# taleinat/fuzzysearch

Measured on NVIDIA H100. Metric: haystack_GB_per_s_scanned, higher is better.
Workload: dtype u8

## Files before the change

### fuzzysearch_b200/csrc/api.cu

```cuda
#include <algorithm>
#include <atomic>
#include <cstdarg>
#include <cstdio>
#include <cmath>
#include <cstring>
#include <dlfcn.h>
#include <sched.h>
#include <unistd.h>
#include <condition_variable>
#include <memory>
#include <mutex>
#include <thread>
#include <new>
#include <string>
#include <type_traits>
#include <vector>

#include "kernels.cuh"
#include "ham_kernels.cuh"
#include "lp_kernels.cuh"
#include "post_kernels.cuh"
#include "p2p_kernels.cuh"
#include "batch_kernels.cuh"
#include "ham_batch_kernels.cuh"
// ... 163 lines not shown
    int (*CommInitRank)(void **comm, int nranks, NcclId id, int rank) = nullptr;
    int (*AllGather)(const void *send, void *recv, size_t count, int dtype, void *comm, cudaStream_t s) = nullptr;
    int (*CommDestroy)(void *comm) = nullptr;
    const char *(*GetErrorString)(int) = nullptr;
    bool ok = false;
};
static NcclApi g_nccl;
static std::string g_nccl_path;

extern "C" void fzb_nccl_set_library(const char *path) { g_nccl_path = path ? path : ""; }

static int nccl_load() {
    static std::once_flag once;
    std::call_once(once, [] {
        void *lib = nullptr;
        if (!g_nccl_path.empty()) lib = dlopen(g_nccl_path.c_str(), RTLD_NOW | RTLD_GLOBAL);
        if (!lib) lib = dlopen("libnccl.so.2", RTLD_NOW | RTLD_GLOBAL);
        if (!lib) lib = dlopen("libnccl.so", RTLD_NOW | RTLD_GLOBAL);
        if (!lib) return;
        *(void **)&g_nccl.GetUniqueId = dlsym(lib, "ncclGetUniqueId");
        *(void **)&g_nccl.CommInitRank = dlsym(lib, "ncclCommInitRank");
        *(void **)&g_nccl.AllGather = dlsym(lib, "ncclAllGather");
        *(void **)&g_nccl.CommDestroy = dlsym(lib, "ncclCommDestroy");
        *(void **)&g_nccl.GetErrorString = dlsym(lib, "ncclGetErrorString");
        g_nccl.ok = g_nccl.GetUniqueId && g_nccl.CommInitRank && g_nccl.AllGather && g_nccl.CommDestroy;
    });
    return g_nccl.ok ? FZB_OK : fail(FZB_E_CUDA, "libnccl.so.2 not available: %s", dlerror() ? dlerror() : "missing symbols");
}

static void nccl_comm_destroy(void *comm) {
    if (g_nccl.ok && comm) g_nccl.CommDestroy(comm);
}

#define NCCLCK(call)                                                                                      \
    do {                                                                                                  \
        int r_ = (call);                                                                                  \
        if (r_ != 0)                                                                                      \
            return fail(FZB_E_CUDA, "%s failed: %s", #call, g_nccl.GetErrorString ? g_nccl.GetErrorString(r_) : "?"); \
    } while (0)

struct fzb_haystack {
    std::recursive_mutex mu;
    int device = 0;
    uint8_t *d = nullptr;
    DevBuf<uint8_t> owned_buf;
    uint64_t buf_len = 0, buf_lo = 0, global_len = 0, own_lo = 0, own_hi = 0;
    uint64_t padded_len = 0;
    cudaEvent_t ev_stop = nullptr;
    cudaStream_t stream = nullptr;
    DevBuf<uint32_t> d_bitmap;
    DevBuf<RawRec> d_out;
    DevBuf<uint32_t> d_counters;
    MappedBuf<uint32_t> h_counters;
    MappedBuf<int64_t> h_fin;
    DevBuf<int64_t> d_fin;
    DevBuf<uint64_t> d_sorted;
    fzb_result *pending = nullptr;
    bool ev1_recorded = false;
    bool filter_attrs_set = false;
    int scan_per_sm = 0;
    double coll_prob = -1.0;
    bool p2p = false;
    bool local_world = false;
    std::unique_ptr<PeerBufs> peer;
    uint8_t *peer_base[kMaxWorld] = {};
    bool peer_opened[kMaxWorld] = {};
    uint32_t p2p_cap = 4096;
    uint64_t slot_bytes = 0, flags_off = 0;
    uint32_t epoch = 0;
    bool counters_clean = false;
    uint32_t seq = 0;
    void *comm = nullptr;
    int rank = 0, world = 1;
    uint32_t gather_cap = 4096;
    std::unique_ptr<GatherBufs> gather;
    cudaEvent_t ev[4] = {nullptr, nullptr, nullptr, nullptr};
    int sm_count = 132;
    DevBuf<uint64_t> d_hits;
    DevBuf<uint32_t> d_glist;
    uint32_t glist_cap = 0;
    DevBuf<uint32_t> d_scratch;
    DevBuf<unsigned long long> d_lplist;
    std::unique_ptr<BatchBufs> batch;
    DevBuf<unsigned long long> d_mhits;
    std::unique_ptr<LpBatchBufs> lpb;
    std::unique_ptr<GenericBatchBufs> gbatch;
    std::unique_ptr<RecBufs> recs;
    std::unique_ptr<BestBufs> bestb;
    std::unique_ptr<NearBufs> nearb;
    std::unique_ptr<NearBatchBufs> nearbatch;
};

struct fzb_result {
    std::vector<RawRec> raw;
    uint32_t raw_n = 0;
    fzb_haystack *owner = nullptr;
    bool raw_in_stage = false;
    void fetch_raw();
    void discard_attempt();
    std::vector<RawRec> fin;
    std::vector<int64_t> hulls;
    bool unconsolidated = false;
    bool have_fin = false;
    bool device_post = false;
    bool raw_ordered = false;
    bool has_global = false;
    bool global_on_device = false;
    bool fused_issued = false;
    uint32_t fused_status = 0;
    uint32_t gcount = 0;
    std::vector<RawRec> gfin;
    int raw_order = 0;
    void order_raw();
    fzb_stats stats{};
};

static uint64_t round_up(uint64_t x, uint64_t a) { return (x + a - 1) / a * a; }

static RawRec make_rec(int64_t start, int64_t end, int64_t dist) {
    RawRec r;
    r.start = start;
    r.end = end;
    r.dist = (int32_t)dist;
    r.idx = -1;
    r.ngram = -1;
    return r;
}

struct HandleLock {
    std::recursive_mutex *m;
    explicit HandleLock(fzb_haystack *h) : m(h ? &h->mu : nullptr) {
        if (m) m->lock();
    }
    ~HandleLock() {
        if (m) m->unlock();
    }
    HandleLock(const HandleLock &) = delete;
    HandleLock &operator=(const HandleLock &) = delete;
};

static std::mutex g_pending_mutex;

void fzb_result::fetch_raw() {
    std::lock_guard<std::mutex> lock(g_pending_mutex);
    if (!owner) return;
    if (raw_in_stage) {
        raw.resize(raw_n);
        if (raw_n) {
            cudaSetDevice(owner->device);
            if (cudaMemcpyAsync(raw.data(), owner->d_out.get(), (size_t)raw_n * sizeof(RawRec), cudaMemcpyDeviceToHost,
                                owner->stream) != cudaSuccess ||
                cudaStreamSynchronize(owner->stream) != cudaSuccess) {
                cudaGetLastError();
                raw.clear();
                raw_n = 0;
            }
        }
        raw_in_stage = false;
    }
    if (global_on_device) {
        gfin.resize(gcount);
        for (uint32_t i = 0; i < gcount; i++) {
            const int64_t s0 = owner->peer->h_grows[2 * (size_t)i], v = owner->peer->h_grows[2 * (size_t)i + 1];
            gfin[i] = make_rec(s0, s0 + (v >> 32), v & 0xFFFFFFFF);
        }
        global_on_device = false;
    }
    owner->pending = nullptr;
    owner = nullptr;
}

void fzb_result::discard_attempt() {
    fetch_raw();
    raw.clear();
    raw_n = 0;
    fin.clear();
}

static void detach_pending(fzb_haystack *h) {
    fzb_result *r;
    {
        std::lock_guard<std::mutex> lock(g_pending_mutex);
        r = h->pending;
    }
    if (r) r->fetch_raw();
}

static int alloc_out(fzb_haystack *h, uint64_t cap) { return h->d_out.alloc(cap, cap * (sizeof(RawRec) + sizeof(uint64_t))); }

static int haystack_common_init(fzb_haystack *h) {
    CK(cudaSetDevice(h->device));
    CK(cudaStreamCreateWithFlags(&h->stream, cudaStreamNonBlocking));
    for (auto &e : h->ev) CK(cudaEventCreate(&e));
    CK(cudaEventCreate(&h->ev_stop));
    cudaDeviceProp prop;
    CK(cudaGetDeviceProperties(&prop, h->device));
    h->sm_count = prop.multiProcessorCount;
    uint64_t granules = (h->padded_len >> kGranuleShift) + 2;
    TRY(h->d_bitmap.alloc(round_up((granules + 31) / 32, 32)));
    TRY(h->d_counters.alloc(CNT_COUNT));
    TRY(h->h_counters.alloc(CNT_COUNT));
    memset(h->h_counters.get(), 0, CNT_COUNT * sizeof(uint32_t));
    TRY(h->h_fin.alloc((uint64_t)kPostMax * kFinCols));
    TRY(h->d_fin.alloc((uint64_t)kPostMax * kFinCols));
    TRY(h->d_sorted.alloc(kPostMax));
    CK(cudaFuncSetAttribute(k_post, cudaFuncAttributeMaxDynamicSharedMemorySize, (int)kPostSmem));
    CK(cudaMemset(h->d_bitmap.get(), 0, h->d_bitmap.size() * sizeof(uint32_t)));
    h->glist_cap = (uint32_t)std::min<uint64_t>(granules, 1u << 20);
    TRY(h->d_glist.alloc(std::max<uint32_t>(h->glist_cap, 1)));
    return alloc_out(h, 1u << 16);
}

static int check_shard(uint64_t buf_len, uint64_t buf_lo, uint64_t global_len, uint64_t own_lo,
                       uint64_t own_hi) {
    if (global_len >= (1ull << 46)) return fail(FZB_E_INVALID, "global_len must be below 2^46");
    if (buf_lo > global_len || buf_len > global_len - buf_lo || own_lo > own_hi || own_hi > global_len ||
        (own_lo < own_hi && (own_lo < buf_lo || own_hi > buf_lo + buf_len)))
        return fail(FZB_E_INVALID, "inconsistent shard geometry");
    if (buf_lo % 16 != 0) return fail(FZB_E_INVALID, "buf_lo must be a multiple of 16");
    if (buf_len >= (1ull << 40)) return fail(FZB_E_INVALID, "buf_len must be below 2^40");
    return FZB_OK;
}

static int alloc_buffer(fzb_haystack *h) {
    CK(cudaSetDevice(h->device));
    TRY(h->owned_buf.alloc(h->padded_len));
    h->d = h->owned_buf.get();
    CK(cudaMemset(h->d + h->buf_len, 0, h->padded_len - h->buf_len));
    return FZB_OK;
}

static void close_peers(fzb_haystack *h);
static int upload_bytes(fzb_haystack *h, uint64_t dst_off, const uint8_t *host, uint64_t n);

extern "C" void fzb_haystack_destroy(fzb_haystack *h) {
    if (!h) return;
    cudaSetDevice(h->device);
    if (h->stream) cudaStreamSynchronize(h->stream);
    detach_pending(h);
    if (h->comm) nccl_comm_destroy(h->comm);
    close_peers(h);
    for (auto &e : h->ev)
        if (e) cudaEventDestroy(e);
    if (h->ev_stop) cudaEventDestroy(h->ev_stop);
    if (h->stream) cudaStreamDestroy(h->stream);
    delete h;
}

static int haystack_new(const char *arg_error, const uint8_t *host, const void *dev_ptr, uint64_t buf_len,
                        uint64_t buf_lo, uint64_t global_len, uint64_t own_lo, uint64_t own_hi, int device,
                        fzb_haystack **out) {
    if (!out) return fail(FZB_E_INVALID, "out is NULL");
    *out = nullptr;
    if (arg_error) return fail(FZB_E_INVALID, "%s", arg_error);
    int rc = check_shard(buf_len, buf_lo, global_len, own_lo, own_hi);
    if (rc) return rc;
// ... 640 lines not shown
    uint64_t n = 0;
    for (uint64_t c : counts) n += c;
    std::vector<GroupRow> g;
    g.reserve(n);
    for (uint64_t c : counts) {
        const size_t seam = g.size();
        for (uint64_t i = 0; i < c; i++, rows += kFinCols) g.push_back(GroupRow{rows[0], rows[1], rows[2], rows[3], rows[4]});
        if (!std::is_sorted(g.begin() + seam, g.end(), group_less)) std::sort(g.begin() + seam, g.end(), group_less);
        if (seam > 0 && seam < g.size() && group_less(g[seam], g[seam - 1])) {
            auto lo = std::upper_bound(g.begin(), g.begin() + seam, g[seam], group_less);
            auto hi = std::lower_bound(g.begin() + seam, g.end(), g[seam - 1], group_less);
            std::inplace_merge(lo, g.begin() + seam, hi, group_less);
        }
    }
    if (!std::is_sorted(g.begin(), g.end(), group_less)) std::sort(g.begin(), g.end(), group_less);
    return g;
}

static void write_group_rows(const std::vector<RawRec> &fin, const std::vector<int64_t> &hulls, size_t n, int64_t *rows) {
    for (size_t i = 0; i < n; i++, rows += kFinCols) {
        rows[0] = fin[i].start;
        rows[1] = fin[i].end;
        rows[2] = fin[i].dist;
        rows[3] = hulls[2 * i];
        rows[4] = hulls[2 * i + 1];
    }
}

extern "C" int64_t fzb_consolidate(const int64_t *start, const int64_t *end, const int32_t *dist, uint64_t n,
                                   int64_t *out_start, int64_t *out_end, int32_t *out_dist) {
    if (n && (!start || !end || !dist)) return fail(FZB_E_INVALID, "NULL input");
    std::vector<RawRec> o;
    sweep_groups(match_rows(start, end, dist, n), o);
    for (size_t i = 0; i < o.size(); i++) {
        if (out_start) out_start[i] = o[i].start;
        if (out_end) out_end[i] = o[i].end;
        if (out_dist) out_dist[i] = o[i].dist;
    }
    return (int64_t)o.size();
}

extern "C" int64_t fzb_consolidate_groups(const int64_t *start, const int64_t *end, const int32_t *dist, uint64_t n,
                                          int64_t *out_rows) {
    if (n && (!start || !end || !dist || !out_rows)) return fail(FZB_E_INVALID, "NULL input");
    std::vector<RawRec> o;
    std::vector<int64_t> hulls;
    sweep_groups(match_rows(start, end, dist, n), o, &hulls);
    write_group_rows(o, hulls, o.size(), out_rows);
    return (int64_t)o.size();
}

extern "C" int64_t fzb_result_group_rows(const fzb_result *r, int64_t *rows, uint64_t max_rows) {
    if (!r || (!rows && max_rows)) return fail(FZB_E_INVALID, "NULL argument");
    if (!r->have_fin || r->hulls.size() != r->fin.size() * 2)
        return fail(FZB_E_INVALID, "result was produced with FZB_F_NO_FINAL");
    write_group_rows(r->fin, r->hulls, std::min<size_t>(r->fin.size(), max_rows), rows);
    return (int64_t)r->fin.size();
}

extern "C" int fzb_result_hulls(const fzb_result *r, int64_t *hull_start, int64_t *hull_end) {
    if (!r) return fail(FZB_E_INVALID, "result is NULL");
    if (!r->have_fin || r->hulls.size() != r->fin.size() * 2)
        return fail(FZB_E_INVALID, "result was produced with FZB_F_NO_FINAL");
    for (size_t i = 0; i < r->fin.size(); i++) {
        if (hull_start) hull_start[i] = r->hulls[2 * i];
        if (hull_end) hull_end[i] = r->hulls[2 * i + 1];
    }
    return FZB_OK;
}

extern "C" int64_t fzb_merge_groups(const int64_t *rows, uint64_t n, int64_t *out_start, int64_t *out_end,
                                    int32_t *out_dist) {
    if (n && !rows) return fail(FZB_E_INVALID, "NULL input");
    std::vector<RawRec> o;
    sweep_groups(read_group_runs(rows, {n}), o);
    for (size_t i = 0; i < o.size(); i++) {
        if (out_start) out_start[i] = o[i].start;
        if (out_end) out_end[i] = o[i].end;
        if (out_dist) out_dist[i] = o[i].dist;
    }
    return (int64_t)o.size();
}

static int allgather_groups_staged(fzb_haystack *h, const std::vector<int64_t> &rows, std::vector<int64_t> &all,
                                   std::vector<uint64_t> &counts) {
    const uint64_t n = rows.size() / kFinCols;
    for (;;) {
        const uint32_t cap = h->gather_cap;
        TRY(ensure_gather_buffers(h, cap));
        GatherBufs &g = *h->gather;
        const size_t slot_rows = (size_t)cap + 1, slot = slot_rows * kFinCols * sizeof(int64_t);
        g.h_send[0] = (int64_t)n;
        g.h_send[1] = n <= cap;
        g.h_send[2] = g.h_send[3] = g.h_send[4] = 0;
        if (n <= cap && n) memcpy(g.h_send.get() + kFinCols, rows.data(), n * kFinCols * sizeof(int64_t));
        CK(cudaMemcpyAsync(g.d_send.get(), g.h_send.get(), (1 + (n <= cap ? n : 0)) * kFinCols * sizeof(int64_t),
                           cudaMemcpyHostToDevice, h->stream));
        NCCLCK(g_nccl.AllGather(g.d_send.get(), g.d_recv.get(), slot,  0, h->comm, h->stream));
        CK(cudaMemcpyAsync(g.h_recv.get(), g.d_recv.get(), slot * h->world, cudaMemcpyDeviceToHost, h->stream));
        CK(cudaStreamSynchronize(h->stream));
        uint64_t top = 0;
        for (int r = 0; r < h->world; r++) top = std::max<uint64_t>(top, (uint64_t)g.h_recv[(size_t)r * slot_rows * kFinCols]);
        if (top <= cap) {
            all.clear();
            counts.clear();
            for (int r = 0; r < h->world; r++) {
                const int64_t *base = g.h_recv.get() + (size_t)r * slot_rows * kFinCols;
                all.insert(all.end(), base + kFinCols, base + kFinCols + (size_t)base[0] * kFinCols);
                counts.push_back((uint64_t)base[0]);
            }
            return FZB_OK;
        }
        while (h->gather_cap < top) h->gather_cap *= 2;
    }
// ... 109 lines not shown

constexpr uint64_t kMaxRawRecs = 1ull << 27;

static int ensure_out_cap(fzb_haystack *h, uint64_t need) {
    if (need <= h->d_out.size()) return FZB_OK;
    uint64_t cap = h->d_out.size();
    while (cap < need) cap *= 2;
    if (cap > kMaxRawRecs) return fail(FZB_E_UNSUPPORTED, "more than 2^27 raw matches in one search");
    return alloc_out(h, cap);
}


static int wait_done(fzb_haystack *h, const volatile uint32_t *word) {
    const uint32_t want = h->seq;
    for (uint64_t spins = 0; *word != want; spins++) {
#if defined(__x86_64__) || defined(__i386__)
        __builtin_ia32_pause();
#endif
        if ((spins & 0xFFF) == 0xFFF) {
            const cudaError_t e = cudaStreamQuery(h->stream);
            if (e == cudaSuccess) break;
            if (e != cudaErrorNotReady) return fail(FZB_E_CUDA, "search failed: %s", cudaGetErrorString(e));
        }
    }
    std::atomic_thread_fence(std::memory_order_acquire);
    if (*word != want) {
        CK(cudaStreamSynchronize(h->stream));
        CK(cudaGetLastError());
        if (*word != want) return fail(FZB_E_CUDA, "search kernels did not complete");
    }
    return FZB_OK;
}

struct PostPlan {
    int mode = 1;
    bool global = false;
};

static void finalize_on_host(fzb_result *res, int mode);

template <class F>
static int run_emitting(fzb_haystack *h, fzb_result *res, F enqueue, PostPlan post = PostPlan()) {
    detach_pending(h);
    for (int attempt = 0; attempt < 8; attempt++) {
        if (!h->counters_clean) CK(cudaMemsetAsync(h->d_counters.get(), 0, CNT_COUNT * sizeof(uint32_t), h->stream));
        h->counters_clean = false;
        CK(cudaEventRecord(h->ev[0], h->stream));
        h->ev1_recorded = false;
        int rc = enqueue();
        if (rc) return rc;
        CK(cudaGetLastError());
        h->seq++;
        PostArgs pa{reinterpret_cast<const uint64_t *>(h->d_out.get() + h->d_out.size()), (uint32_t)h->d_out.size(), post.mode,
                    h->d_sorted.get(), h->d_fin.get(), h->h_fin.get(), h->h_counters.get(), h->d_counters.get(), h->seq, 0};
        pa.clear = !(post.global && attempt == 0 && h->p2p && !res->fused_issued);
        k_post<<<h->sm_count, kPostThreads, kPostSmem, h->stream>>>(pa);
        CK(cudaGetLastError());
        res->stats.n_launches++;
        const bool fused = post.global && attempt == 0 && h->p2p && !res->fused_issued;
        if (fused) {
            h->epoch++;
            WorldArgs w{};
            w.world = h->world;
            w.rank = h->rank;
            w.epoch = h->epoch;
            w.cap = h->p2p_cap;
            w.slot_bytes = h->slot_bytes;
            w.flags_off = h->flags_off;
            for (int r = 0; r < h->world; r++) w.peer[r] = h->peer_base[r];
            PeerBufs &pb = *h->peer;
            k_push<<<kPushCtas, kPushThreads, 0, h->stream>>>(w, h->d_fin.get(), h->d_counters.get(), post.mode, pb.d_ms.get());
            MergeOut mo{pb.d_mscore.get(), pb.d_mpos.get(), pb.h_grows.get(), pb.h_ghdr.get(), h->seq};
            k_merge<<<h->world, kPostThreads, 0, h->stream>>>(w, pb.d_ms.get(), mo);
            CK(cudaGetLastError());
            res->stats.n_launches += 2;
        }
        CK(cudaEventRecord(h->ev[2], h->stream));
        rc = wait_done(h, fused ? h->peer->h_ghdr.get() + 7 : h->h_counters.get() + CNT_SEQ);
        if (rc) return rc;
        const uint32_t n = h->h_counters[CNT_OUT];
        res->stats.n_candidates = h->h_counters[CNT_CAND];
        if (fused) {
            res->fused_issued = true;
            res->fused_status = h->peer->h_ghdr[0];
            res->gcount = h->peer->h_ghdr[1];
            if (h->peer->h_ghdr[2] != h->epoch && res->fused_status == MS_OK) res->fused_status = MS_TIMEOUT;
        }
        if (n > h->d_out.size()) {
            TRY(ensure_out_cap(h, n));
            continue;
        }
        const bool posted = h->h_counters[CNT_POST_DONE] != 0;
        h->counters_clean = posted && (!fused || (res->fused_status == MS_OK));
        res->raw.clear();
        res->raw_n = n;
        res->raw_ordered = false;
        if (posted || (res->fused_issued && res->fused_status == MS_OK)) {
            std::lock_guard<std::mutex> lock(g_pending_mutex);
            res->raw_in_stage = posted;
            res->owner = h;
            h->pending = res;
        }
        if (!posted && n) {
            res->raw.resize(n);
            CK(cudaMemcpyAsync(res->raw.data(), h->d_out.get(), (size_t)n * sizeof(RawRec), cudaMemcpyDeviceToHost, h->stream));
            CK(cudaStreamSynchronize(h->stream));
        }
        res->fin.clear();
        res->hulls.clear();
        res->have_fin = false;
        res->device_post = false;
        if (post.mode != 0) {
            if (posted) {
                const uint32_t nf = h->h_counters[CNT_NFINAL];
                res->fin.resize(nf);
                res->hulls.resize((size_t)nf * 2);
                for (uint32_t i = 0; i < nf; i++) {
                    res->fin[i] = make_rec(h->h_fin[kFinCols * i], h->h_fin[kFinCols * i + 1], h->h_fin[kFinCols * i + 2]);
                    res->hulls[2 * i] = h->h_fin[kFinCols * i + 3];
                    res->hulls[2 * i + 1] = h->h_fin[kFinCols * i + 4];
                }
                res->device_post = true;
            } else {
                finalize_on_host(res, post.mode);
            }
            res->have_fin = true;
        }
        float ms = 0.f;
        while (cudaEventQuery(h->ev[2]) == cudaErrorNotReady) {
        }
        cudaEventElapsedTime(&ms, h->ev[0], h->ev[2]);
        res->stats.gpu_ms = ms;
        res->stats.filter_ms = ms;
        if (h->ev1_recorded) {
            cudaEventElapsedTime(&ms, h->ev[0], h->ev[1]);
            res->stats.filter_ms = ms;
        }
        return FZB_OK;
    }
    return fail(FZB_E_CUDA, "output buffer kept overflowing");
}

static void sort_generation_order(std::vector<RawRec> &v) {
    std::sort(v.begin(), v.end(), [](const RawRec &a, const RawRec &b) {
        if (a.ngram != b.ngram) return a.ngram < b.ngram;
        return a.idx < b.idx;
    });
}

static void sort_canonical(std::vector<RawRec> &v) {
    std::sort(v.begin(), v.end(), [](const RawRec &a, const RawRec &b) {
        if (a.start != b.start) return a.start < b.start;
        if (a.end != b.end) return a.end < b.end;
        return a.dist < b.dist;
    });
}

void fzb_result::order_raw() {
    fetch_raw();
    if (raw_ordered) return;
    if (raw_order == 0)
        sort_generation_order(raw);
    else if (raw_order == 1)
        sort_canonical(raw);
    else
        std::sort(raw.begin(), raw.end(), [](const RawRec &a, const RawRec &b) {
            if (a.ngram != b.ngram) return a.ngram < b.ngram;
            if (a.idx != b.idx) return a.idx < b.idx;
            if (a.start != b.start) return a.start < b.start;
            if (a.end != b.end) return a.end < b.end;
            return a.dist < b.dist;
        });
    raw_ordered = true;
}

static void finalize_on_host(fzb_result *res, int mode) {
    if (mode == 1) {
        consolidate_recs(res->raw, res->fin, &res->hulls);
        return;
    }
    res->fin = res->raw;
    sort_canonical(res->fin);
    res->hulls.resize(res->fin.size() * 2);
    for (size_t i = 0; i < res->fin.size(); i++) {
        res->fin[i].idx = -1;
        res->fin[i].ngram = -1;
        res->hulls[2 * i] = res->fin[i].start;
        res->hulls[2 * i + 1] = res->fin[i].end;
    }
}

static int set_filter_attrs(size_t smem) {
    CK(cudaFuncSetAttribute(k_filter_sampled, cudaFuncAttributeMaxDynamicSharedMemorySize, (int)smem));
    CK(cudaFuncSetAttribute(k_filter_dense<0>, cudaFuncAttributeMaxDynamicSharedMemorySize, (int)kDenseSmem));
    CK(cudaFuncSetAttribute(k_filter_dense<1>, cudaFuncAttributeMaxDynamicSharedMemorySize, (int)kDenseSmem));
    CK(cudaFuncSetAttribute(k_filter_dense<2>, cudaFuncAttributeMaxDynamicSharedMemorySize, (int)kDenseSmem));
    CK(cudaFuncSetAttribute(k_filter_dense<3>, cudaFuncAttributeMaxDynamicSharedMemorySize, (int)kDenseSmem));
    CK(cudaFuncSetAttribute(k_filter_dense2, cudaFuncAttributeMaxDynamicSharedMemorySize, (int)kDense2Smem));
    return FZB_OK;
}

constexpr int kVerifyCtasPerSm = 8;

static bool sampled_filter_applies(uint32_t m, uint32_t k, uint32_t flags) {
    if (flags & FZB_F_FORCE_DENSE) return false;
    if (m < 4 || m < k + 3) return false;
    return (m - k - 3) / 4 >= k + 1;
}

static int sample_collision_prob(fzb_haystack *h) {
    if (h->coll_prob >= 0.0) return FZB_OK;
    const uint64_t blk = 4096, nblk = 16;
// ... 261 lines not shown
                k_generic_lp<R><<<grid, kLpThreads, 0, h->stream>>>(p, h->d_scratch.get(), cap, h->d_out.get(),
                                                                    h->d_out.size(), h->d_counters.get(), rs);
            });
            res->stats.n_launches++;
            return FZB_OK;
        }, PostPlan{post_mode, post_mode != 0 && (flags & FZB_F_GLOBAL) != 0});
        if (rc) return rc;
        res->raw_order = 1;
        return FZB_OK;
    }
    p.L = (int)pl.L();
    p.n_ngrams = (int)pl.m / p.L;
    const bool sampled = sampled_filter(h, pl, flags);
    p.q = sampled ? 4 : std::min(p.L, 8);
    res->stats.route = 5;
    rc = set_filter_attrs(kScanSmem);
    if (rc) return rc;
    rc = run_lp(h, res, [&](int grid, int cap) -> int {
        int r2 = enqueue_filter(h, p, sampled, res);
        if (r2) return r2;
        with_recs(h, [&](auto rec) {
            constexpr bool R = decltype(rec)::value;
            k_verify_generic<R><<<grid, kLpThreads, 0, h->stream>>>(p, h->d_bitmap.size(), h->d_scratch.get(), cap,
                                                                    h->d_out.get(), h->d_out.size(), h->d_counters.get(), rs);
        });
        res->stats.n_launches++;
        return FZB_OK;
    }, PostPlan{post_mode, post_mode != 0 && (flags & FZB_F_GLOBAL) != 0});
    if (rc) return rc;
    res->raw_order = 2;
    return FZB_OK;
}

static int finish_global(fzb_haystack *h, fzb_result *res) {
    if (h->world < 1 || (!h->comm && !h->local_world))
        return fail(FZB_E_INVALID, "FZB_F_GLOBAL needs fzb_haystack_comm_init / fzb_comm_init_local");
    if (res->fused_issued) {
        if (res->fused_status == MS_OK) {
            res->has_global = true;
            res->global_on_device = true;
            return FZB_OK;
        }
        if (res->fused_status == MS_TIMEOUT)
            return fail(FZB_E_CUDA, "multi-GPU reduction timed out waiting for a peer (rank %d of %d)", h->rank, h->world);
    }
    if (h->local_world && res->fused_issued && res->fused_status == MS_OVERFLOW)
        return fail(FZB_E_UNSUPPORTED, "NCCL-free world: more than %u groups continue across shard seams; the staged "
                    "fallback needs an NCCL communicator (fzb_haystack_comm_init)", kMaxNonHeads);
    if (h->local_world)
        return fail(FZB_E_UNSUPPORTED, "NCCL-free world: a shard produced more than %u groups (or more than %d raw "
                    "matches); the staged fallback needs an NCCL communicator (fzb_haystack_comm_init)", h->p2p_cap, kPostMax);
    std::vector<int64_t> all;
    std::vector<uint64_t> counts;
    std::vector<int64_t> rows(res->fin.size() * kFinCols);
    write_group_rows(res->fin, res->hulls, res->fin.size(), rows.data());
    int rc = allgather_groups_staged(h, rows, all, counts);
    if (rc) return rc;
    if (res->unconsolidated) {
        res->gfin.resize(all.size() / kFinCols);
        for (size_t i = 0; i < res->gfin.size(); i++)
            res->gfin[i] = make_rec(all[kFinCols * i], all[kFinCols * i + 1], all[kFinCols * i + 2]);
        sort_canonical(res->gfin);
    } else {
        sweep_groups(read_group_runs(all.data(), counts), res->gfin);
    }
    res->gcount = (uint32_t)res->gfin.size();
    res->has_global = true;
    return FZB_OK;
}

static int make_result(fzb_result **out, fzb_result **res) {
    if (!out) return fail(FZB_E_INVALID, "out is NULL");
    *out = nullptr;
    *res = new (std::nothrow) fzb_result();
    if (!*res) return fail(FZB_E_CUDA, "out of host memory");
    return FZB_OK;
}

static int search_hamming(fzb_haystack *h, const uint8_t *pattern, const Plan &pl, uint32_t flags, fzb_result *res);

static int run_route(fzb_haystack *h, const uint8_t *pattern, const Plan &pl, uint32_t flags, fzb_result *res) {
    res->unconsolidated = pl.route == Route::Exact || pl.route == Route::Hamming;
    const int post_mode = res->unconsolidated ? 2 : (flags & FZB_F_NO_FINAL) ? 0 : 1;
    int rc = pl.route == Route::Hamming ? search_hamming(h, pattern, pl, flags, res)
             : pl.route == Route::LevLp ? search_lev_lp(h, pattern, pl, flags, res, post_mode)
             : pl.generic()             ? search_generic(h, pattern, pl, flags, res, post_mode)
                                        : search_lev_ngrams(h, pattern, pl, flags, res, post_mode);
    if (rc == FZB_OK && post_mode && (flags & FZB_F_GLOBAL)) rc = finish_global(h, res);
    return rc;
}

template <class P>
static int run_search(fzb_haystack *h, const uint8_t *pattern, uint32_t flags, fzb_result **out, P plan) {
    HandleLock handle_lock(h);
    fzb_result *res;
    int rc = make_result(out, &res);
    if (rc) return rc;
    Plan pl;
    rc = plan(pl);
    if (rc == FZB_OK) rc = run_route(h, pattern, pl, flags, res);
    if (rc) {
        fzb_result_destroy(res);
        return rc;
    }
    *out = res;
    return FZB_OK;
// ... 755 lines not shown
    explicit BufferView(fzb_haystack *hs)
        : h(hs), d(hs->d), buf_len(hs->buf_len), buf_lo(hs->buf_lo), own_lo(hs->own_lo), own_hi(hs->own_hi),
          padded_len(hs->padded_len), global_len(hs->global_len), coll_prob(hs->coll_prob) {}
    ~BufferView() {
        h->d = d;
        h->buf_len = buf_len;
        h->buf_lo = buf_lo;
        h->own_lo = own_lo;
        h->own_hi = own_hi;
        h->padded_len = padded_len;
        h->global_len = global_len;
        h->coll_prob = coll_prob;
    }
    BufferView(const BufferView &) = delete;
    BufferView &operator=(const BufferView &) = delete;
    void set(uint64_t vlo, uint64_t vhi, uint64_t lo, uint64_t hi) {
        h->d = d + (vlo - buf_lo);
        h->buf_lo = vlo;
        h->buf_len = vhi - vlo;
        h->padded_len = round_up(h->buf_len, 128) + 128;
        h->own_lo = lo;
        h->own_hi = hi;
    }
};

extern "C" int fzb_search_exact_window(fzb_haystack *h, const uint8_t *pattern, uint32_t m, uint64_t start,
                                       uint64_t end, uint32_t flags, fzb_result **out) {
    HandleLock handle_lock(h);
    if (!h || !out) return fail(FZB_E_INVALID, "NULL argument");
    *out = nullptr;
    TRY(refuse_records(h, "the windowed exact search"));
    if (flags & FZB_F_GLOBAL) return fail(FZB_E_INVALID, "windowed exact search is per handle");
    if (!is_whole_sequence(h)) return fail(FZB_E_INVALID, "windowed exact search needs a whole (unsharded) sequence");
    start = std::min<uint64_t>(start, h->global_len);
    end = std::max<uint64_t>(start, std::min<uint64_t>(end, h->global_len));
    if (end - start < m) {
        Plan pl;
        int rc0 = plan_exact(h, pattern, m, flags, pl);
        if (rc0) return rc0;
        fzb_result *res;
        rc0 = make_result(out, &res);
        if (rc0) return rc0;
        res->unconsolidated = true;
        res->have_fin = true;
        *out = res;
        return FZB_OK;
    }
    const uint64_t halo = round_up((uint64_t)m, 128) + 128;
    BufferView view(h);
    view.set((start > halo ? start - halo : 0) / 128 * 128, end, start, end);
    h->global_len = end;
    h->coll_prob = -1.0;
    const int rc = fzb_search_exact(h, pattern, m, flags, out);
    if (rc == FZB_OK && *out) (*out)->fetch_raw();
    return rc;
}

typedef CUresult (*EncodeTiledFn)(CUtensorMap *, CUtensorMapDataType, cuuint32_t, void *, const cuuint64_t *,
                                  const cuuint64_t *, const cuuint32_t *, const cuuint32_t *, CUtensorMapInterleave,
                                  CUtensorMapSwizzle, CUtensorMapL2promotion, CUtensorMapFloatOOBfill);

static int make_row_maps(fzb_haystack *h, CUtensorMap *map256, CUtensorMap *map8) {
    static const EncodeTiledFn encode = []() -> EncodeTiledFn {
        void *fn = nullptr;
        cudaDriverEntryPointQueryResult q;
        if (cudaGetDriverEntryPoint("cuTensorMapEncodeTiled", &fn, cudaEnableDefault, &q) != cudaSuccess) return nullptr;
        return (fn && q == cudaDriverEntryPointSuccess) ? (EncodeTiledFn)fn : nullptr;
    }();
    if (!encode) {
        cudaGetLastError();
        return fail(FZB_E_CUDA, "cuTensorMapEncodeTiled not available");
    }
    const cuuint64_t rows = h->padded_len / kHcRowBytes;
    const cuuint64_t dims[2] = {(cuuint64_t)kHcRowBytes, rows};
    const cuuint64_t strides[1] = {(cuuint64_t)kHcRowBytes};
    const cuuint32_t estr[2] = {1, 1};
    for (int which = 0; which < 2; which++) {
        const cuuint32_t box[2] = {(cuuint32_t)kHcRowBytes, which == 0 ? 256u : (cuuint32_t)kHcHaloRows};
        CUresult r = encode(which == 0 ? map256 : map8, CU_TENSOR_MAP_DATA_TYPE_UINT8, 2, h->d, dims, strides, box,
                            estr, CU_TENSOR_MAP_INTERLEAVE_NONE, CU_TENSOR_MAP_SWIZZLE_128B,
                            CU_TENSOR_MAP_L2_PROMOTION_L2_128B, CU_TENSOR_MAP_FLOAT_OOB_FILL_NONE);
        if (r != CUDA_SUCCESS) return fail(FZB_E_CUDA, "cuTensorMapEncodeTiled failed (%d)", (int)r);
    }
    return FZB_OK;
}

static int search_hamming(fzb_haystack *h, const uint8_t *pattern, const Plan &pl, uint32_t flags, fzb_result *res) {
    const uint32_t m = pl.m;
    int rc;
    ScanParams p;
    fill_params(h, pattern, m, p);
    p.k = (int)pl.k;
    if (flags & FZB_F_TINY_LIST) p.glist_cap = std::min(h->glist_cap, 8u);
    const RecSet rs = rec_set(h);
    CK(cudaSetDevice(h->device));
    res->stats.route = 4;
    res->stats.bytes_scanned = h->buf_len;
    const bool counting = !(flags & FZB_F_FORCE_DENSE) && (int)m >= 4 * p.k + 7 && p.k <= 7 && h->buf_len > 0;
    HamCountParams hp{};
    CUtensorMap map256, map8;
    int slices = 0;
    if (counting) {
        hp.Wc = std::min<int>((int)(m - 3) / 4, 8);
        slices = hp.Wc - p.k <= 4 ? 2 : 3;
        hp.bias = (1 << slices) - (hp.Wc - p.k);
        hp.nrows = (int64_t)(round_up(h->buf_len, kHcRowBytes) / kHcRowBytes);
        rc = make_row_maps(h, &map256, &map8);
// ... 931 lines not shown
    } while (rc == FZB_OK && !*found && lo < whole.own_hi);
    return rc;
}

extern "C" int fzb_debug_counters(const fzb_haystack *h, uint32_t out[32]) {
    if (!h || !out) return fail(FZB_E_INVALID, "NULL argument");
    memset(out, 0, 32 * sizeof(uint32_t));
    memcpy(out, h->h_counters.get(), CNT_COUNT * sizeof(uint32_t));
    if (h->peer) memcpy(out + 16, h->peer->h_ghdr.get(), 16 * sizeof(uint32_t));
    return FZB_OK;
}

extern "C" int fzb_debug_expand(const uint8_t *subs, const uint32_t *sub_off, const uint8_t *seqs,
                                const uint32_t *seq_off, const int32_t *max_l, const int32_t *variant, uint32_t count,
                                int device, int32_t *out) {
    if (count && (!subs || !sub_off || !seqs || !seq_off || !max_l || !variant || !out))
        return fail(FZB_E_INVALID, "NULL argument");
    if (device < 0 || device >= fzb_device_count()) return fail(FZB_E_CUDA, "CUDA device %d not available", device);
    if (count == 0) return FZB_OK;
    for (uint32_t i = 0; i < count; i++) {
        if (sub_off[i + 1] < sub_off[i] || seq_off[i + 1] < seq_off[i]) return fail(FZB_E_INVALID, "bad offsets");
        if (sub_off[i + 1] - sub_off[i] >= (uint32_t)kDbgMax || seq_off[i + 1] - seq_off[i] >= 2u * kDbgMax)
            return fail(FZB_E_UNSUPPORTED, "case %u too long for the debug entry", i);
        if (variant[i] < 0 || variant[i] > 2 || max_l[i] < 0) return fail(FZB_E_INVALID, "bad variant / budget");
    }
    CK(cudaSetDevice(device));
    const size_t nsub = std::max<size_t>(sub_off[count], 1), nseq = std::max<size_t>(seq_off[count], 1);
    DevBuf<uint8_t> d_subs, d_seqs;
    DevBuf<uint32_t> d_so, d_qo;
    DevBuf<int32_t> d_k, d_v, d_out;
    TRY(d_subs.alloc(nsub));
    TRY(d_seqs.alloc(nseq));
    TRY(d_so.alloc(count + 1));
    TRY(d_qo.alloc(count + 1));
    TRY(d_k.alloc(count));
    TRY(d_v.alloc(count));
    TRY(d_out.alloc((uint64_t)count * 8));
    CK(cudaMemcpy(d_subs.get(), subs, sub_off[count], cudaMemcpyHostToDevice));
    CK(cudaMemcpy(d_seqs.get(), seqs, seq_off[count], cudaMemcpyHostToDevice));
    CK(cudaMemcpy(d_so.get(), sub_off, (count + 1) * sizeof(uint32_t), cudaMemcpyHostToDevice));
    CK(cudaMemcpy(d_qo.get(), seq_off, (count + 1) * sizeof(uint32_t), cudaMemcpyHostToDevice));
    CK(cudaMemcpy(d_k.get(), max_l, count * sizeof(int32_t), cudaMemcpyHostToDevice));
    CK(cudaMemcpy(d_v.get(), variant, count * sizeof(int32_t), cudaMemcpyHostToDevice));
    k_debug_expand<<<count, 32>>>(d_subs.get(), d_so.get(), d_seqs.get(), d_qo.get(), d_k.get(), d_v.get(), d_out.get());
    CK(cudaGetLastError());
    CK(cudaMemcpy(out, d_out.get(), (size_t)count * 8 * sizeof(int32_t), cudaMemcpyDeviceToHost));
    return FZB_OK;
}

extern "C" uint64_t fzb_result_count(const fzb_result *r, int which) {
    if (!r) return 0;
    if (which != FZB_RAW && r->has_global) return r->gcount;
    if (which == FZB_RAW) return r->raw_n;
    return r->fin.size();
}

extern "C" int fzb_result_copy(const fzb_result *r, int which, int64_t *start, int64_t *end, int32_t *dist,
                               int32_t *anchor_ngram, int64_t *anchor_idx) {
    if (!r) return fail(FZB_E_INVALID, "result is NULL");
    if (which == FZB_RAW) const_cast<fzb_result *>(r)->order_raw();
    if (which != FZB_RAW && r->has_global) const_cast<fzb_result *>(r)->fetch_raw();
    const std::vector<RawRec> &v = (which != FZB_RAW && r->has_global) ? r->gfin : (which == FZB_RAW ? r->raw : r->fin);
    const bool anchors = (which == FZB_RAW) && (r->stats.route <= 2);
    for (size_t i = 0; i < v.size(); i++) {
        if (start) start[i] = v[i].start;
        if (end) end[i] = v[i].end;
        if (dist) dist[i] = v[i].dist;
        if (anchor_ngram) anchor_ngram[i] = anchors ? v[i].ngram : -1;
        if (anchor_idx) anchor_idx[i] = anchors ? v[i].idx : -1;
    }
    return FZB_OK;
}

extern "C" int fzb_result_stats(const fzb_result *r, fzb_stats *out) {
    if (!r || !out) return fail(FZB_E_INVALID, "NULL argument");
    *out = r->stats;
    return FZB_OK;
}

extern "C" void fzb_result_destroy(fzb_result *r) {
    if (!r) return;
    {
        std::lock_guard<std::mutex> lock(g_pending_mutex);
        if (r->owner) {
            r->owner->pending = nullptr;
            r->owner = nullptr;
        }
    }
    delete r;
}
```

### fuzzysearch_b200/csrc/post_kernels.cuh

```cuda
#pragma once
#include "kernels.cuh"

namespace fzb {

constexpr int kPostMax = 16384;
constexpr int kPostThreads = 1024;
enum { CNT_POST_DONE = 5, CNT_NFINAL = 6, CNT_TICKET = 9, CNT_SEQ = 15 };
constexpr int kFinCols = 5;
constexpr size_t kPostSmem = (size_t)kPostMax * 8 + (size_t)kPostMax * 4;

struct PostArgs {
    const uint64_t *rkeys;
    uint32_t cap;
    int mode;
    uint64_t *sorted;
    int64_t *fin;
    int64_t *h_fin;
    uint32_t *h_counters;
    uint32_t *counters;
    uint32_t seq;
    int clear;
};

__device__ __forceinline__ uint32_t gtimer_lo() {
#ifdef FZB_EMU
    return (uint32_t)emu::cycles();
#else
    unsigned long long t;
    asm volatile("mov.u64 %0, %globaltimer;" : "=l"(t));
    return (uint32_t)t;
#endif
}

__device__ __forceinline__ uint32_t block_scan_sum(uint32_t v, uint32_t *scratch, uint32_t *total) {
    const int lane = threadIdx.x & 31, w = threadIdx.x >> 5;
    uint32_t inc = v;
#pragma unroll
    for (int o = 1; o < 32; o <<= 1) {
        const uint32_t t = __shfl_up_sync(0xFFFFFFFFu, inc, o);
        if (lane >= o) inc += t;
    }
    if (lane == 31) scratch[w] = inc;
    __syncthreads();
    if (w == 0) {
        const uint32_t x = scratch[lane];
        uint32_t xi = x;
#pragma unroll
        for (int o = 1; o < 32; o <<= 1) {
            const uint32_t t = __shfl_up_sync(0xFFFFFFFFu, xi, o);
            if (lane >= o) xi += t;
        }
        scratch[lane] = xi - x;
        if (lane == 31) scratch[32] = xi;
    }
    __syncthreads();
    const uint32_t r = scratch[w] + inc - v;
    *total = scratch[32];
    __syncthreads();
    return r;
}

__device__ __forceinline__ unsigned long long block_scan_max(unsigned long long v, unsigned long long *scratch,
                                                             unsigned long long *total) {
    const int lane = threadIdx.x & 31, w = threadIdx.x >> 5;
    unsigned long long inc = v;
#pragma unroll
    for (int o = 1; o < 32; o <<= 1) {
        const unsigned long long t = __shfl_up_sync(0xFFFFFFFFu, inc, o);
        if (lane >= o) inc = max(inc, t);
    }
// ... 31 lines not shown
    __shared__ uint32_t s_ticket;
    const uint32_t nraw = a.counters[CNT_OUT];
    const uint32_t n = a.counters[CNT_KEYS];
    const bool fits = nraw <= (uint32_t)kPostMax && nraw <= a.cap;
    const uint32_t tid = threadIdx.x, lane = tid & 31, warp = tid >> 5;
    const uint32_t G = gridDim.x, b = blockIdx.x;
    if (!fits) {
        if (b == 0) {
            if (tid < CNT_SEQ) a.h_counters[tid] = a.counters[tid];
            __threadfence_system();
            __syncthreads();
            if (tid == 0) a.h_counters[CNT_SEQ] = a.seq;
        }
        return;
    }
    const uint32_t t_start = gtimer_lo();
    const uint32_t lo = (uint32_t)((uint64_t)n * b / G), hi = (uint32_t)((uint64_t)n * (b + 1) / G);
    if (a.mode != 0 && n > 0) {
        for (uint32_t i = tid; i < n; i += kPostThreads) keys[i] = a.rkeys[i];
        __syncthreads();
        for (uint32_t i0 = lo + 2 * warp; i0 < hi; i0 += 2 * (kPostThreads / 32)) {
            const uint32_t i1 = min(i0 + 1, hi - 1);
            const uint64_t key0 = keys[i0], key1 = keys[i1];
            uint32_t c0 = 0, c1 = 0;
            for (uint32_t j = lane; j < n; j += 32) {
                const uint64_t kj = keys[j];
                c0 += (kj < key0) || (kj == key0 && j < i0);
                c1 += (kj < key1) || (kj == key1 && j < i1);
            }
            c0 = __reduce_add_sync(0xFFFFFFFFu, c0);
            c1 = __reduce_add_sync(0xFFFFFFFFu, c1);
            if (lane == 0) {
                a.sorted[c0] = key0;
                a.sorted[c1] = key1;
            }
        }
    }
    const uint32_t t_ranked = gtimer_lo();
    __threadfence();
    __syncthreads();
    if (tid == 0) s_ticket = atomicAdd(&a.counters[CNT_TICKET], 1u);
    __syncthreads();
    if (s_ticket != G - 1) return;
    __threadfence();
    const uint32_t t_ticket = gtimer_lo();
    uint32_t t_sorted = t_ticket, t_swept = t_ticket;
    uint32_t nfinal = 0;
    if (a.mode != 0 && n > 0) {
        for (uint32_t i = tid; i < n; i += kPostThreads) keys[i] = __ldcg(a.sorted + i);
        __syncthreads();
        t_sorted = gtimer_lo();
        if (a.mode == 2) {
            nfinal = n;
            for (uint32_t i = tid; i < n; i += kPostThreads) {
                const uint64_t kx = keys[i];
                const int64_t s = (int64_t)(kx >> 18), e = s + (int64_t)((kx >> 8) & 1023u);
                int64_t *row = a.fin + (size_t)kFinCols * i;
                row[0] = s;
                row[1] = e;
                row[2] = (int64_t)(kx & 255u);
                row[3] = s;
                row[4] = e;
            }
        } else {
            for (uint32_t i = tid; i < n; i += kPostThreads) segbest[i] = 0xFFFFFFFFu;
            __syncthreads();
            unsigned long long carry_hull = 0;
            uint32_t carry_groups = 0;
            for (uint32_t base = 0; base < n; base += kPostThreads) {
                const uint32_t i = base + tid;
                const bool live = i < n;
                const uint64_t kx = live ? keys[i] : 0;
                const unsigned long long s = kx >> 18, len = (kx >> 8) & 1023u, e = live ? s + len : 0;
                unsigned long long round_max;
                const unsigned long long hull = max(carry_hull, block_scan_max(e, scr64, &round_max));
                const bool head = live && (i == 0 || s >= hull);
                uint32_t round_heads;
                const uint32_t before = block_scan_sum(head ? 1u : 0u, scr32, &round_heads);
                if (live) {
                    const uint32_t g = carry_groups + before + (head ? 1u : 0u) - 1u;
                    if (head) {
                        a.fin[(size_t)kFinCols * g + 3] = (int64_t)s;
                        if (g >= 1) a.fin[(size_t)kFinCols * (g - 1) + 4] = (int64_t)hull;
                    }
                    if (i == n - 1) a.fin[(size_t)kFinCols * g + 4] = (int64_t)max(hull, e);
                    const uint32_t score = ((uint32_t)(kx & 255u) << 24) | ((uint32_t)(1023u - len) << 14) | i;
                    atomicMin(&segbest[g], score);
                }
                carry_hull = max(carry_hull, round_max);
                carry_groups += round_heads;
            }
            nfinal = carry_groups;
            __syncthreads();
            for (uint32_t g = tid; g < nfinal; g += kPostThreads) {
                const uint64_t kx = keys[segbest[g] & 16383u];
                const int64_t s = (int64_t)(kx >> 18);
                int64_t *row = a.fin + (size_t)kFinCols * g;
                row[0] = s;
                row[1] = s + (int64_t)((kx >> 8) & 1023u);
                row[2] = (int64_t)(kx & 255u);
            }
        }
        __threadfence_block();
        __syncthreads();
        t_swept = gtimer_lo();
        const uint32_t nvec = (uint32_t)(((size_t)nfinal * kFinCols * 8 + 15) / 16);
        const uint4 *src = reinterpret_cast<const uint4 *>(a.fin);
        uint4 *dst = reinterpret_cast<uint4 *>(a.h_fin);
        for (uint32_t i = tid; i < nvec; i += kPostThreads) dst[i] = __ldcg(src + i);
    }
    __syncthreads();
    if (tid == 0) {
        a.counters[CNT_NFINAL] = nfinal;
        a.counters[CNT_POST_DONE] = 1u;
        a.counters[10] = t_ranked - t_start;
        a.counters[11] = t_sorted - t_ranked;
        a.counters[12] = t_swept - t_sorted;
        a.counters[13] = gtimer_lo() - t_swept;
    }
    __syncthreads();
    if (tid < CNT_SEQ) a.h_counters[tid] = a.counters[tid];
    if (a.clear && tid < CNT_COUNT) a.counters[tid] = 0;
    __threadfence_system();
    __syncthreads();
    if (tid == 0) a.h_counters[CNT_SEQ] = a.seq;
}

}
```

Measured before the change: 2782.

## Stage compact keys to host and defer hull rows fetch lazily

The post kernel now writes one packed 64-bit key per final match to mapped host memory, replacing the 5-column int64 rows it used to copy. Hull rows stay in device memory and are pulled only when a caller asks for groups or hulls. Result decoding on the host is deferred until first access. The segment sweep is also changed from many block-wide scan rounds to one chunked per-thread pass with a single max-scan and sum-scan, cutting __syncthreads rounds. The cost is extra complexity in the lazy fetch state and a synchronous device copy when hulls are requested.

```diff
diff --git a/fuzzysearch_b200/csrc/api.cu b/fuzzysearch_b200/csrc/api.cu
--- a/fuzzysearch_b200/csrc/api.cu
+++ b/fuzzysearch_b200/csrc/api.cu
@@ -239,7 +239,7 @@
     DevBuf<RawRec> d_out;
     DevBuf<uint32_t> d_counters;
     MappedBuf<uint32_t> h_counters;
-    MappedBuf<int64_t> h_fin;
+    MappedBuf<uint64_t> h_keys;
     DevBuf<int64_t> d_fin;
     DevBuf<uint64_t> d_sorted;
     fzb_result *pending = nullptr;
@@ -278,15 +278,20 @@
     std::unique_ptr<NearBatchBufs> nearbatch;
 };
 
+enum : unsigned { STAGED_RAW = 1, STAGED_FIN = 2, STAGED_HULLS = 4, STAGED_GLOBAL = 8, STAGED_ALL = 15 };
+
 struct fzb_result {
     std::vector<RawRec> raw;
     uint32_t raw_n = 0;
     fzb_haystack *owner = nullptr;
     bool raw_in_stage = false;
-    void fetch_raw();
+    void fetch(unsigned parts);
     void discard_attempt();
     std::vector<RawRec> fin;
     std::vector<int64_t> hulls;
+    uint32_t fin_n = 0;
+    bool fin_in_stage = false;
+    bool hulls_in_stage = false;
     bool unconsolidated = false;
     bool have_fin = false;
     bool device_post = false;
@@ -328,10 +333,10 @@
 
 static std::mutex g_pending_mutex;
 
-void fzb_result::fetch_raw() {
+void fzb_result::fetch(unsigned parts) {
     std::lock_guard<std::mutex> lock(g_pending_mutex);
     if (!owner) return;
-    if (raw_in_stage) {
+    if ((parts & STAGED_RAW) && raw_in_stage) {
         raw.resize(raw_n);
         if (raw_n) {
             cudaSetDevice(owner->device);
@@ -345,7 +350,35 @@
         }
         raw_in_stage = false;
     }
-    if (global_on_device) {
+    if ((parts & STAGED_FIN) && fin_in_stage) {
+        fin.resize(fin_n);
+        for (uint32_t i = 0; i < fin_n; i++) {
+            const uint64_t kx = owner->h_keys[i];
+            const int64_t s0 = (int64_t)(kx >> 18);
+            fin[i] = make_rec(s0, s0 + (int64_t)((kx >> 8) & 1023u), (int64_t)(kx & 255u));
+        }
+        fin_in_stage = false;
+    }
+    if ((parts & STAGED_HULLS) && hulls_in_stage) {
+        std::vector<int64_t> rows((size_t)fin_n * kFinCols);
+        hulls.assign((size_t)fin_n * 2, 0);
+        if (fin_n) {
+            cudaSetDevice(owner->device);
+            if (cudaMemcpyAsync(rows.data(), owner->d_fin.get(), rows.size() * sizeof(int64_t), cudaMemcpyDeviceToHost,
+                                owner->stream) != cudaSuccess ||
+                cudaStreamSynchronize(owner->stream) != cudaSuccess) {
+                cudaGetLastError();
+                hulls.clear();
+            } else {
+                for (uint32_t i = 0; i < fin_n; i++) {
+                    hulls[2 * (size_t)i] = rows[(size_t)kFinCols * i + 3];
+                    hulls[2 * (size_t)i + 1] = rows[(size_t)kFinCols * i + 4];
+                }
+            }
+        }
+        hulls_in_stage = false;
+    }
+    if ((parts & STAGED_GLOBAL) && global_on_device) {
         gfin.resize(gcount);
         for (uint32_t i = 0; i < gcount; i++) {
             const int64_t s0 = owner->peer->h_grows[2 * (size_t)i], v = owner->peer->h_grows[2 * (size_t)i + 1];
@@ -353,12 +386,14 @@
         }
         global_on_device = false;
     }
-    owner->pending = nullptr;
-    owner = nullptr;
+    if (!raw_in_stage && !fin_in_stage && !hulls_in_stage && !global_on_device) {
+        owner->pending = nullptr;
+        owner = nullptr;
+    }
 }
 
 void fzb_result::discard_attempt() {
-    fetch_raw();
+    fetch(STAGED_ALL);
     raw.clear();
     raw_n = 0;
     fin.clear();
@@ -370,7 +405,7 @@
         std::lock_guard<std::mutex> lock(g_pending_mutex);
         r = h->pending;
     }
-    if (r) r->fetch_raw();
+    if (r) r->fetch(STAGED_ALL);
 }
 
 static int alloc_out(fzb_haystack *h, uint64_t cap) { return h->d_out.alloc(cap, cap * (sizeof(RawRec) + sizeof(uint64_t))); }
@@ -388,7 +423,7 @@
     TRY(h->d_counters.alloc(CNT_COUNT));
     TRY(h->h_counters.alloc(CNT_COUNT));
     memset(h->h_counters.get(), 0, CNT_COUNT * sizeof(uint32_t));
-    TRY(h->h_fin.alloc((uint64_t)kPostMax * kFinCols));
+    TRY(h->h_keys.alloc(kPostMax));
     TRY(h->d_fin.alloc((uint64_t)kPostMax * kFinCols));
     TRY(h->d_sorted.alloc(kPostMax));
     CK(cudaFuncSetAttribute(k_post, cudaFuncAttributeMaxDynamicSharedMemorySize, (int)kPostSmem));
@@ -1135,6 +1170,7 @@
 
 extern "C" int64_t fzb_result_group_rows(const fzb_result *r, int64_t *rows, uint64_t max_rows) {
     if (!r || (!rows && max_rows)) return fail(FZB_E_INVALID, "NULL argument");
+    const_cast<fzb_result *>(r)->fetch(STAGED_FIN | STAGED_HULLS);
     if (!r->have_fin || r->hulls.size() != r->fin.size() * 2)
         return fail(FZB_E_INVALID, "result was produced with FZB_F_NO_FINAL");
     write_group_rows(r->fin, r->hulls, std::min<size_t>(r->fin.size(), max_rows), rows);
@@ -1143,6 +1179,7 @@
 
 extern "C" int fzb_result_hulls(const fzb_result *r, int64_t *hull_start, int64_t *hull_end) {
     if (!r) return fail(FZB_E_INVALID, "result is NULL");
+    const_cast<fzb_result *>(r)->fetch(STAGED_FIN | STAGED_HULLS);
     if (!r->have_fin || r->hulls.size() != r->fin.size() * 2)
         return fail(FZB_E_INVALID, "result was produced with FZB_F_NO_FINAL");
     for (size_t i = 0; i < r->fin.size(); i++) {
@@ -1358,7 +1395,7 @@
         CK(cudaGetLastError());
         h->seq++;
         PostArgs pa{reinterpret_cast<const uint64_t *>(h->d_out.get() + h->d_out.size()), (uint32_t)h->d_out.size(), post.mode,
-                    h->d_sorted.get(), h->d_fin.get(), h->h_fin.get(), h->h_counters.get(), h->d_counters.get(), h->seq, 0};
+                    h->d_sorted.get(), h->d_fin.get(), h->h_keys.get(), h->h_counters.get(), h->d_counters.get(), h->seq, 0};
         pa.clear = !(post.global && attempt == 0 && h->p2p && !res->fused_issued);
         k_post<<<h->sm_count, kPostThreads, kPostSmem, h->stream>>>(pa);
         CK(cudaGetLastError());
@@ -1418,14 +1455,8 @@
         res->device_post = false;
         if (post.mode != 0) {
             if (posted) {
-                const uint32_t nf = h->h_counters[CNT_NFINAL];
-                res->fin.resize(nf);
-                res->hulls.resize((size_t)nf * 2);
-                for (uint32_t i = 0; i < nf; i++) {
-                    res->fin[i] = make_rec(h->h_fin[kFinCols * i], h->h_fin[kFinCols * i + 1], h->h_fin[kFinCols * i + 2]);
-                    res->hulls[2 * i] = h->h_fin[kFinCols * i + 3];
-                    res->hulls[2 * i + 1] = h->h_fin[kFinCols * i + 4];
-                }
+                res->fin_n = h->h_counters[CNT_NFINAL];
+                res->fin_in_stage = res->hulls_in_stage = true;
                 res->device_post = true;
             } else {
                 finalize_on_host(res, post.mode);
@@ -1463,7 +1494,7 @@
 }
 
 void fzb_result::order_raw() {
-    fetch_raw();
+    fetch(STAGED_RAW);
     if (raw_ordered) return;
     if (raw_order == 0)
         sort_generation_order(raw);
@@ -1831,6 +1862,7 @@
                     "matches); the staged fallback needs an NCCL communicator (fzb_haystack_comm_init)", h->p2p_cap, kPostMax);
     std::vector<int64_t> all;
     std::vector<uint64_t> counts;
+    res->fetch(STAGED_FIN | STAGED_HULLS);
     std::vector<int64_t> rows(res->fin.size() * kFinCols);
     write_group_rows(res->fin, res->hulls, res->fin.size(), rows.data());
     int rc = allgather_groups_staged(h, rows, all, counts);
@@ -2692,7 +2724,7 @@
     h->global_len = end;
     h->coll_prob = -1.0;
     const int rc = fzb_search_exact(h, pattern, m, flags, out);
-    if (rc == FZB_OK && *out) (*out)->fetch_raw();
+    if (rc == FZB_OK && *out) (*out)->fetch(STAGED_ALL);
     return rc;
 }
 
@@ -3730,14 +3762,14 @@
     if (!r) return 0;
     if (which != FZB_RAW && r->has_global) return r->gcount;
     if (which == FZB_RAW) return r->raw_n;
-    return r->fin.size();
+    return r->fin_in_stage ? r->fin_n : r->fin.size();
 }
 
 extern "C" int fzb_result_copy(const fzb_result *r, int which, int64_t *start, int64_t *end, int32_t *dist,
                                int32_t *anchor_ngram, int64_t *anchor_idx) {
     if (!r) return fail(FZB_E_INVALID, "result is NULL");
     if (which == FZB_RAW) const_cast<fzb_result *>(r)->order_raw();
-    if (which != FZB_RAW && r->has_global) const_cast<fzb_result *>(r)->fetch_raw();
+    if (which != FZB_RAW) const_cast<fzb_result *>(r)->fetch(r->has_global ? STAGED_GLOBAL : STAGED_FIN);
     const std::vector<RawRec> &v = (which != FZB_RAW && r->has_global) ? r->gfin : (which == FZB_RAW ? r->raw : r->fin);
     const bool anchors = (which == FZB_RAW) && (r->stats.route <= 2);
     for (size_t i = 0; i < v.size(); i++) {
diff --git a/fuzzysearch_b200/csrc/post_kernels.cuh b/fuzzysearch_b200/csrc/post_kernels.cuh
--- a/fuzzysearch_b200/csrc/post_kernels.cuh
+++ b/fuzzysearch_b200/csrc/post_kernels.cuh
@@ -15,7 +15,7 @@
     int mode;
     uint64_t *sorted;
     int64_t *fin;
-    int64_t *h_fin;
+    uint64_t *h_keys;
     uint32_t *h_counters;
     uint32_t *counters;
     uint32_t seq;
@@ -153,62 +153,59 @@
         t_sorted = gtimer_lo();
         if (a.mode == 2) {
             nfinal = n;
-            for (uint32_t i = tid; i < n; i += kPostThreads) {
+        } else {
+            for (uint32_t i = tid; i < n; i += kPostThreads) segbest[i] = 0xFFFFFFFFu;
+            const uint32_t R = ((n + kPostThreads - 1) / kPostThreads) | 1u;
+            const uint32_t i0 = min(n, tid * R), i1 = min(n, i0 + R);
+            unsigned long long emax = 0;
+            for (uint32_t i = i0; i < i1; i++) {
                 const uint64_t kx = keys[i];
-                const int64_t s = (int64_t)(kx >> 18), e = s + (int64_t)((kx >> 8) & 1023u);
-                int64_t *row = a.fin + (size_t)kFinCols * i;
-                row[0] = s;
-                row[1] = e;
-                row[2] = (int64_t)(kx & 255u);
+                emax = max(emax, (unsigned long long)((kx >> 18) + ((kx >> 8) & 1023u)));
+            }
+            unsigned long long all_max;
+            const unsigned long long hull_in = block_scan_max(emax, scr64, &all_max);
+            uint32_t heads = 0;
+            unsigned long long hull = hull_in;
+            for (uint32_t i = i0; i < i1; i++) {
+                const uint64_t kx = keys[i];
+                const unsigned long long s = kx >> 18;
+                heads += (i == 0 || s >= hull) ? 1u : 0u;
+                hull = max(hull, s + ((kx >> 8) & 1023u));
+            }
+            const uint32_t before = block_scan_sum(heads, scr32, &nfinal);
+            uint32_t g = before - 1u, best = 0xFFFFFFFFu;
+            hull = hull_in;
+            for (uint32_t i = i0; i < i1; i++) {
+                const uint64_t kx = keys[i];
+                const unsigned long long s = kx >> 18, len = (kx >> 8) & 1023u, e = s + len;
+                if (i == 0 || s >= hull) {
+                    if (best != 0xFFFFFFFFu) atomicMin(&segbest[g], best);
+                    best = 0xFFFFFFFFu;
+                    g++;
+                    a.fin[(size_t)kFinCols * g + 3] = (int64_t)s;
+                    if (g >= 1) a.fin[(size_t)kFinCols * (g - 1) + 4] = (int64_t)hull;
+                }
+                if (i == n - 1) a.fin[(size_t)kFinCols * g + 4] = (int64_t)max(hull, e);
+                best = min(best, ((uint32_t)(kx & 255u) << 24) | ((uint32_t)(1023u - len) << 14) | i);
+                hull = max(hull, e);
+            }
+            if (best != 0xFFFFFFFFu) atomicMin(&segbest[g], best);
+            __syncthreads();
+        }
+        t_swept = gtimer_lo();
+        for (uint32_t g = tid; g < nfinal; g += kPostThreads) {
+            const uint64_t kx = a.mode == 2 ? keys[g] : keys[segbest[g] & 16383u];
+            const int64_t s = (int64_t)(kx >> 18), e = s + (int64_t)((kx >> 8) & 1023u);
+            int64_t *row = a.fin + (size_t)kFinCols * g;
+            row[0] = s;
+            row[1] = e;
+            row[2] = (int64_t)(kx & 255u);
+            if (a.mode == 2) {
                 row[3] = s;
                 row[4] = e;
             }
-        } else {
-            for (uint32_t i = tid; i < n; i += kPostThreads) segbest[i] = 0xFFFFFFFFu;
-            __syncthreads();
-            unsigned long long carry_hull = 0;
-            uint32_t carry_groups = 0;
-            for (uint32_t base = 0; base < n; base += kPostThreads) {
-                const uint32_t i = base + tid;
-                const bool live = i < n;
-                const uint64_t kx = live ? keys[i] : 0;
-                const unsigned long long s = kx >> 18, len = (kx >> 8) & 1023u, e = live ? s + len : 0;
-                unsigned long long round_max;
-                const unsigned long long hull = max(carry_hull, block_scan_max(e, scr64, &round_max));
-                const bool head = live && (i == 0 || s >= hull);
-                uint32_t round_heads;
-                const uint32_t before = block_scan_sum(head ? 1u : 0u, scr32, &round_heads);
-                if (live) {
-                    const uint32_t g = carry_groups + before + (head ? 1u : 0u) - 1u;
-                    if (head) {
-                        a.fin[(size_t)kFinCols * g + 3] = (int64_t)s;
-                        if (g >= 1) a.fin[(size_t)kFinCols * (g - 1) + 4] = (int64_t)hull;
-                    }
-                    if (i == n - 1) a.fin[(size_t)kFinCols * g + 4] = (int64_t)max(hull, e);
-                    const uint32_t score = ((uint32_t)(kx & 255u) << 24) | ((uint32_t)(1023u - len) << 14) | i;
-                    atomicMin(&segbest[g], score);
-                }
-                carry_hull = max(carry_hull, round_max);
-                carry_groups += round_heads;
-            }
-            nfinal = carry_groups;
-            __syncthreads();
-            for (uint32_t g = tid; g < nfinal; g += kPostThreads) {
-                const uint64_t kx = keys[segbest[g] & 16383u];
-                const int64_t s = (int64_t)(kx >> 18);
-                int64_t *row = a.fin + (size_t)kFinCols * g;
-                row[0] = s;
-                row[1] = s + (int64_t)((kx >> 8) & 1023u);
-                row[2] = (int64_t)(kx & 255u);
-            }
-        }
-        __threadfence_block();
-        __syncthreads();
-        t_swept = gtimer_lo();
-        const uint32_t nvec = (uint32_t)(((size_t)nfinal * kFinCols * 8 + 15) / 16);
-        const uint4 *src = reinterpret_cast<const uint4 *>(a.fin);
-        uint4 *dst = reinterpret_cast<uint4 *>(a.h_fin);
-        for (uint32_t i = tid; i < nvec; i += kPostThreads) dst[i] = __ldcg(src + i);
+            a.h_keys[g] = kx;
+        }
     }
     __syncthreads();
     if (tid == 0) {
```

Measured after the change: 2822 (median of 6 runs). No clear change (+1.4%).
